# alexncoleman/WeaklySupervisedDL

Hardware: AMD Instinct MI355X
Metric: SegmentationModel train img/s at B=16 256x256 (higher is better)
Workload: dtype f32

## Files before the change

### weaklysuperviseddl_amd/csrc/conv_igemm.hip

```cpp
#include "common.h"

#include <type_traits>
#include <algorithm>
#include <cstdint>
#include <mutex>

typedef float f32x16 __attribute__((ext_vector_type(16)));

namespace {

constexpr int kThreads = 256;

struct ConvSrc {
    const float* x;
    const float* wt;
    const float* x_amax;
    int KH, KW, bh, ch, K, Cin;
    long long x_bs;
    unsigned x_bytes;
};

struct ConvP {
    const float* x;
    const float* wt;
// ... 2182 lines not shown
            }
        }
        __syncthreads();
    }
    float* slab = p.slab + (long long)blockIdx.x * 64 * 147;
#pragma unroll
    for (int r = 0; r < 16; ++r) {
        const int row = (r & 3) + 8 * (r >> 2) + 4 * lh;
        const int n = nt0 * 32 + l31;
        if (n < 147) {
            slab[(long long)row * 147 + n] = acc0[r];
            slab[(long long)(32 + row) * 147 + n] = acc1[r];
        }
        if (third && 128 + l31 < 147) slab[(long long)(wid * 32 + row) * 147 + 128 + l31] = acc2[r];
    }
}

static bool stem_wgrad_eligible(int B, int Cin, int H, int W, int Cout, int kh, int kw, int stride, int pad, int dil) {
    return Cin == 3 && Cout == 64 && kh == 7 && kw == 7 && stride == 2 && pad == 3 && dil == 1 && H >= 7 && W >= 7;
}
static int stem_wgrad_grid(int B, int OH, int OW) {
    const long long tiles = (long long)B * wsdl::cdiv(OH, kSwTH) * wsdl::cdiv(OW, kStemTW);
    return (int)std::min<long long>(tiles, kSwMaxGrid);
}

static size_t wgrad_dys_bytes(int Cout, int Cin, int N, int P) {
    if (!wgrad_chunk32(Cout, Cin, N)) return 0;
    const size_t n = (size_t)wsdl::cdiv(P, 32) * Cout * w2row_bytes(g_conv_arith);
    return n < (1ull << 31) ? n : 0;
}

static int wgrad_bands(int Cout, int Cin, int OW, int W, int kw, int stride, int pad, int dil, Band* bands) {
    int BM, BN;
    bool fast;
    wgrad_tile(Cout, Cin, &BM, &BN, &fast);
    bands[0] = Band{0, OW};
    if (!fast || stride != 1) return 1;
    if (wgrad_chunk32(Cout, Cin, kw * kw * Cin)) return 1;
    return column_bands(OW, W, 1, dil, -pad, 1, kw, bands);
}

size_t wsdl_conv2d_wgrad_presplit_bytes(int B, int Cin, int H, int W, int Cout, int kh, int kw, int stride, int pad, int dil) {
    int OH, OW;
    if (check_geom(B, Cin, H, W, Cout, kh, kw, stride, pad, dil, &OH, &OW)) return 0;
    if (g_conv_arith != 1 && g_conv_arith != 2) return 0;
    if (wgrad_role_swap(Cin, Cout, kh, kw, stride, pad)) return 0;
    const int N = kh * kw * Cin, P = B * OH * OW;
    const size_t bytes = wgrad_dys_bytes(Cout, Cin, N, P);
    if (!bytes || P % 32 != 0) return 0;
    const long long xb = (long long)B * Cin * H * W * 4, dyb = (long long)B * Cout * OH * OW * 4;
    if (xb >= (1ll << 31) || dyb >= (1ll << 31)) return 0;
    bool taps_aligned = true;
    for (int kx = 0; kx < kw; ++kx) taps_aligned = taps_aligned && (((kx * dil - pad) & 3) == 0);
    const bool direct = g_wgrad_direct && taps_aligned && stride == 1 && OW % 32 == 0 && W % 4 == 0 && (H * W) % 4 == 0;
    const bool dyraw = direct && g_wgrad_dyraw && (N / 128 <= 10 || g_wgrad_dyraw == 2) && (OH * OW) % 4 == 0;
    return dyraw ? 0 : bytes;
}

size_t wsdl_conv2d_wgrad_workspace(int B, int Cin, int H, int W, int Cout, int kh, int kw, int stride,
                                   int pad, int dil) {
    int OH, OW;
    if (check_geom(B, Cin, H, W, Cout, kh, kw, stride, pad, dil, &OH, &OW)) return 0;
    if (wgrad_role_swap(Cin, Cout, kh, kw, stride, pad))
        return wsdl::align_up((size_t)Cout * Cin * sizeof(float), 256) +
               wsdl_conv2d_wgrad_workspace(B, Cout, OH, OW, Cin, 1, 1, 1, 0, 1);
    const int N = kh * kw * Cin;
    Band bands[8];
    const int nb = wgrad_bands(Cout, Cin, OW, W, kw, stride, pad, dil, bands);
    const int n_live = __builtin_popcountll(live_taps(H, W, OH, OW, kh, kw, stride, pad, dil)) * Cin;
    size_t slabs = (size_t)nb * wgrad_splits(Cout, Cin, N, B * OH * OW, n_live, wgrad_tap_balance(H, OH, kh, stride, pad, dil)) *
                   Cout * N * sizeof(float);
    if (stem_wgrad_eligible(B, Cin, H, W, Cout, kh, kw, stride, pad, dil))
        slabs = std::max(slabs, (size_t)stem_wgrad_grid(B, OH, OW) * Cout * N * sizeof(float));
    return wsdl::align_up(slabs, 256) + wsdl::align_up(wgrad_dys_bytes(Cout, Cin, N, B * OH * OW), 256) +
           (g_wgrad_chan_scale ? wsdl::align_up((size_t)(Cin + Cout) * sizeof(float), 256) : 0);
}

struct WgradExtra {
    const float* x_chan;
    const float* dy_chan;
    const void* dy_presplit;
};
static int wgrad_impl(const float* x, const float* dy, float* dw, int B, int Cin, int H, int W,
                      int Cout, int kh, int kw, int stride, int pad, int dil, int accumulate,
                      long long x_bs, long long dy_bs, const float* x_amax, const float* dy_amax, void* ws,
                      size_t ws_bytes, wsdl_stream_t stream, WgradExtra ex = WgradExtra{}) {
    WSDL_REQUIRE(x && dy && dw && ws, "conv2d_wgrad: null pointer");
    int OH, OW;
    if (int rc = check_geom(B, Cin, H, W, Cout, kh, kw, stride, pad, dil, &OH, &OW)) return rc;
    if (wgrad_role_swap(Cin, Cout, kh, kw, stride, pad)) {
        const size_t t_bytes = wsdl::align_up((size_t)Cout * Cin * sizeof(float), 256);
        WSDL_REQUIRE(ws_bytes > t_bytes, "conv2d_wgrad: workspace too small");
        float* dwt = static_cast<float*>(ws);
        if (int rc = wgrad_impl(dy, x, dwt, B, Cout, OH, OW, Cin, 1, 1, 1, 0, 1, 0,
                                dy_bs ? dy_bs : (long long)Cout * OH * OW, x_bs ? x_bs : (long long)Cin * H * W,
                                dy_amax, x_amax, static_cast<char*>(ws) + t_bytes, ws_bytes - t_bytes, stream,
                                WgradExtra{ex.dy_chan, ex.x_chan, nullptr}))
            return rc;
        WSDL_TRACE("role-swapped (dW^T) + transpose");
        hipLaunchKernelGGL(transpose_add_kernel, dim3(wsdl::cdiv(Cout, 32), wsdl::cdiv(Cin, 32)), dim3(32, 8), 0,
                           wsdl::as_stream(stream), dwt, dw, Cout, Cin, accumulate);
        WSDL_LAUNCH_CHECK();
        return WSDL_OK;
    }
    WgradP p{};
    p.x = x; p.dy = dy; p.slab = static_cast<float*>(ws);
    p.B = B; p.Cin = Cin; p.H = H; p.W = W; p.Cout = Cout; p.OH = OH; p.OW = OW; p.KH = kh; p.KW = kw;
// ... 37 lines not shown
        return wgrad_reduce_one(rd, s);
    }
    const unsigned long long live_all = live_taps(H, W, OH, OW, kh, kw, stride, pad, dil);
    const int S = wgrad_splits(Cout, Cin, p.N, p.P, __builtin_popcountll(live_all) * Cin, wgrad_tap_balance(H, OH, kh, stride, pad, dil));
    Band bands[8];
    const int nb = wgrad_bands(Cout, Cin, OW, W, kw, stride, pad, dil, bands);
    if (nb == 1) bands[0] = Band{0, OW};
    const int S_total = nb * S;
    p.ow0 = 0; p.own = OW; p.slab0 = 0; p.nb = 1; p.splits = S;
    const size_t need = (size_t)S_total * Cout * p.N * sizeof(float);
    if (ws_bytes < need) {
        wsdl::set_error("conv2d_wgrad: workspace %zu < %zu bytes", ws_bytes, need);
        return WSDL_EWORKSPACE;
    }
    const int chunks = wsdl::cdiv(p.P, 32);
    p.chunks_per_split = wsdl::cdiv(chunks, S);
    hipStream_t s = wsdl::as_stream(stream);
    const long long xb = ((long long)(B - 1) * p.x_bs + (long long)Cin * H * W) * 4;
    const long long dyb = ((long long)(B - 1) * p.dy_bs + (long long)Cout * OH * OW) * 4;
    int tBM, tBN;
    bool fast;
    wgrad_tile(Cout, Cin, &tBM, &tBN, &fast);
    if (fast && (xb >= (1ll << 31) || dyb >= (1ll << 31))) {
        const long long img = std::max((long long)Cin * H * W, (long long)Cout * OH * OW) * 4;
        const long long bs = std::max(p.x_bs, p.dy_bs) * 4;
        WSDL_REQUIRE(B > 1 && img < (1ll << 31), "conv2d_wgrad: a single image of 2 GiB or more is not supported");
        long long per = ((1ll << 31) - 4 - img) / bs + 1;
        if (per < 1) per = 1;
        for (int b0 = 0; b0 < B; b0 += (int)per) {
            const int nb_img = (int)std::min<long long>(per, B - b0);
            if (int rc = wgrad_impl(x + (long long)b0 * p.x_bs, dy + (long long)b0 * p.dy_bs, dw, nb_img, Cin, H, W,
                                    Cout, kh, kw, stride, pad, dil, (accumulate || b0 > 0) ? 1 : 0, p.x_bs, p.dy_bs,
                                    x_amax, dy_amax, ws, ws_bytes, stream, WgradExtra{ex.x_chan, ex.dy_chan, nullptr}))
                return rc;
        }
        return WSDL_OK;
    }
    unsigned long long live_mask = ~0ull;
    {
        const double flops = 2.0 * p.P * (double)Cout * p.N;
        double executed = flops;
        const size_t dys_bytes = fast ? wgrad_dys_bytes(Cout, Cin, p.N, p.P) : 0;
        const size_t dys_off = wsdl::align_up(need, 256);
        const bool chunk32 = dys_bytes && ws_bytes >= dys_off + dys_bytes;
        if (wsdl::prof_enabled() && fast) {
            executed = 0.0;
            for (int i = 0; i < nb; ++i)
                executed += flops * ((double)bands[i].own / OW) *
                            wgrad_executed_fraction(B * OH * bands[i].own, OH, bands[i].ow0, bands[i].own, H, W, kh, kw,
                                                    stride, pad, dil, chunk32 ? 32 : 16);
        }
        bool taps_aligned = true;
        for (int kx = 0; kx < kw; ++kx) taps_aligned = taps_aligned && (((kx * dil - pad) & 3) == 0);
        const bool direct = chunk32 && g_conv_arith && g_wgrad_direct && taps_aligned &&
                            stride == 1 && OW % 32 == 0 && W % 4 == 0 && (H * W) % 4 == 0 && p.x_bs % 4 == 0 &&
                            reinterpret_cast<uintptr_t>(x) % 16 == 0;
        wsdl::ProfScope prof(direct ? WSDL_PROF_WGRAD_SPLIT16D
                                    : chunk32 ? WSDL_PROF_WGRAD_SPLIT32
                                     : fast ? WSDL_PROF_WGRAD_FAST_128x128
                                            : (Cout <= 64 ? WSDL_PROF_WGRAD_64x128 : WSDL_PROF_WGRAD_128x128),
                             s, flops, executed,
                             4.0 * ((double)B * Cin * H * W + (double)p.P * Cout + (double)S_total * Cout * p.N));
        constexpr size_t lds64 = 2 * (64 + 128) * 33 * sizeof(float), lds128 = 2 * (128 + 128) * 33 * sizeof(float);
        static std::once_flag once;
        static hipError_t attr_rc = hipSuccess;
        std::call_once(once, [] {
            attr_rc = hipFuncSetAttribute(reinterpret_cast<const void*>(&conv_wgrad_kernel<64, 128, 1>),
                                          hipFuncAttributeMaxDynamicSharedMemorySize, (int)lds64);
            if (attr_rc == hipSuccess)
                attr_rc = hipFuncSetAttribute(reinterpret_cast<const void*>(&conv_wgrad_kernel<128, 128, 2>),
                                              hipFuncAttributeMaxDynamicSharedMemorySize, (int)lds128);
        });
        WSDL_HIP_CHECK(attr_rc);
        if (fast) {
            p.x_bytes = (unsigned)xb;
            p.dy_bytes = (unsigned)dyb;
            if (chunk32) {
                live_mask = live_all;
                unsigned char* dys = static_cast<unsigned char*>(ws) + dys_off;
                const long long total = 2ll * wsdl::cdiv(p.P, 32) * Cout;
                dim3 grid(p.N / 128, Cout / 128, S);
                p.xcd_order = ((long long)grid.x * grid.y * grid.z) % 8 == 0 ? g_wgrad_xcd : 0;
                const dim3 sgrid((int)std::min<long long>((total + 255) / 256, 16384));
                const size_t cm_off = wsdl::align_up(dys_off + dys_bytes, 256);
                const bool cm_fits = ws_bytes >= cm_off + (size_t)(Cin + Cout) * sizeof(float);
                p.xa_stride = 0;
                int dy_stride = 0;
                if (g_conv_arith) {
                    float* cm = reinterpret_cast<float*>(static_cast<unsigned char*>(ws) + cm_off);
                    if (ex.x_chan) {
                        p.x_amax = x_amax = ex.x_chan;
                        p.xa_stride = 1;
                    } else if (g_wgrad_chan_scale && cm_fits) {
                        WSDL_HIP_CHECK(hipMemsetAsync(cm, 0, (size_t)Cin * sizeof(float), s));
                        hipLaunchKernelGGL(channel_amax_kernel, dim3(Cin, std::min(B, std::max(1, 1024 / Cin))), dim3(256), 0, s, x, B, Cin,
                                           H * W, p.x_bs, cm);
                        WSDL_LAUNCH_CHECK();
                        p.x_amax = x_amax = cm;
                        p.xa_stride = 1;
                    }
                    if (ex.dy_chan) {
                        dy_amax = ex.dy_chan;
                        dy_stride = 1;
                    } else if (g_wgrad_chan_scale && cm_fits) {
                        WSDL_HIP_CHECK(hipMemsetAsync(cm + Cin, 0, (size_t)Cout * sizeof(float), s));
                        hipLaunchKernelGGL(channel_amax_kernel, dim3(Cout, std::min(B, std::max(1, 1024 / Cout))), dim3(256), 0, s, dy, B,
                                           Cout, OH * OW, p.dy_bs, cm + Cin);
                        WSDL_LAUNCH_CHECK();
                        dy_amax = cm + Cin;
                        dy_stride = 1;
                    }
                }
                p.da_stride = dy_stride;
                const bool cs = p.xa_stride || dy_stride;
                const bool presplit = ex.dy_presplit && ex.dy_chan && g_conv_arith;
                if (presplit) dys = static_cast<unsigned char*>(const_cast<void*>(ex.dy_presplit));
                if (g_conv_arith) {
                    WSDL_REQUIRE(x_amax && dy_amax, "conv2d_wgrad: the fp16x2 split kernel needs x_amax and dy_amax");
                    WSDL_TRACE("wgrad_split16%s S=%d xcd=%d cs=%d grid=%ux%ux%u", direct ? "d" : "", S, p.xcd_order, (int)cs, grid.x, grid.y, grid.z);
                    if (direct) {
                        const bool dyraw = !presplit && taps_aligned && g_wgrad_dyraw && (p.N / 128 <= 10 || g_wgrad_dyraw == 2) &&
                                           (OH * OW) % 4 == 0 && p.dy_bs % 4 == 0 &&
                                           reinterpret_cast<uintptr_t>(dy) % 16 == 0 && p.dy_bytes != 0;
                        WSDL_TRACE(dyraw ? "dyraw" : presplit ? "dY pre-split by its producer" : "dy_split16");
                        if (!dyraw && !presplit) {
                            hipLaunchKernelGGL(dy_split16_kernel, sgrid, dim3(256), 0, s, dy, dys, B, Cout, OH * OW, p.dy_bs, p.P, dy_amax,
                                               dy_stride);
                            WSDL_LAUNCH_CHECK();
                        }
                        if (dyraw && cs)
                            hipLaunchKernelGGL((conv_wgrad_split16d_kernel<0, true, true>), grid, dim3(kThreads), 0, s, p, dys,
                                               (unsigned)dys_bytes, dy_amax);
                        else if (dyraw)
                            hipLaunchKernelGGL((conv_wgrad_split16d_kernel<0, true>), grid, dim3(kThreads), 0, s, p, dys,
                                               (unsigned)dys_bytes, dy_amax);
                        else if (cs)
                            hipLaunchKernelGGL((conv_wgrad_split16d_kernel<0, false, true>), grid, dim3(kThreads), 0, s, p, dys,
                                               (unsigned)dys_bytes, dy_amax);
                        else
                            hipLaunchKernelGGL(conv_wgrad_split16d_kernel<0>, grid, dim3(kThreads), 0, s, p, dys,
                                               (unsigned)dys_bytes, dy_amax);
                    } else {
                        WSDL_TRACE(presplit ? "dY pre-split by its producer" : "dy_split16");
                        if (!presplit) {
                            hipLaunchKernelGGL(dy_split16_kernel, sgrid, dim3(256), 0, s, dy, dys, B, Cout, OH * OW, p.dy_bs, p.P, dy_amax,
                                               dy_stride);
                            WSDL_LAUNCH_CHECK();
                        }
                        if (cs)
                            hipLaunchKernelGGL((conv_wgrad_split16_kernel<128, 128, true>), grid, dim3(kThreads), 0, s, p, dys,
                                               (unsigned)dys_bytes, dy_amax);
                        else
                            hipLaunchKernelGGL((conv_wgrad_split16_kernel<128, 128>), grid, dim3(kThreads), 0, s, p, dys,
                                               (unsigned)dys_bytes, dy_amax);
                    }
                } else {
                    WSDL_TRACE("wgrad_split32 bf16x3 S=%d xcd=%d grid=%ux%ux%u", S, p.xcd_order, grid.x, grid.y, grid.z);
                    hipLaunchKernelGGL(dy_split_kernel<0>, sgrid, dim3(256), 0, s, dy, dys, B, Cout, OH * OW, p.dy_bs, p.P,
                                       static_cast<const float*>(nullptr));
                    WSDL_LAUNCH_CHECK();
                    hipLaunchKernelGGL((conv_wgrad_split32_kernel<128, 128, 0>), grid, dim3(kThreads), 0, s, p, dys,
                                       (unsigned)dys_bytes, static_cast<const float*>(nullptr));
                }
            } else {
                WgradP q = p;
                q.nb = nb;
                q.splits = S;
                for (int i = 0; i < nb && nb > 1; ++i) {
                    q.b_ow0[i] = bands[i].ow0;
                    q.b_own[i] = bands[i].own;
                    q.b_cps[i] = wsdl::cdiv(wsdl::cdiv((long long)B * OH * bands[i].own, 32), S);
                }
                int rc;
                WSDL_TRACE("wgrad_fp32_fast<%d,%d> S=%d nb=%d", tBM, tBN, S, nb);
                if (tBM == 128 && tBN == 128) rc = launch_wgrad_fast<128, 128, 2>(q, s, S_total);
                else if (tBM == 128) rc = launch_wgrad_fast<128, 64, 2>(q, s, S_total);
                else if (tBN == 128) rc = launch_wgrad_fast<64, 128, 1>(q, s, S_total);
                else rc = launch_wgrad_fast<64, 64, 2>(q, s, S_total);
                if (rc) return rc;
            }
        } else if (Cout <= 64) {
            WSDL_TRACE("wgrad_fp32_generic<64,128> S=%d", S);
            dim3 grid(wsdl::cdiv(p.N, 128), wsdl::cdiv(Cout, 64), S);
            hipLaunchKernelGGL((conv_wgrad_kernel<64, 128, 1>), grid, dim3(kThreads), lds64, s, p);
        } else {
            WSDL_TRACE("wgrad_fp32_generic<128,128> S=%d", S);
            dim3 grid(wsdl::cdiv(p.N, 128), wsdl::cdiv(Cout, 128), S);
            hipLaunchKernelGGL((conv_wgrad_kernel<128, 128, 2>), grid, dim3(kThreads), lds128, s, p);
        }
    }
    WSDL_LAUNCH_CHECK();
    WgradReduce rd{};
    rd.slab = p.slab; rd.dw = dw; rd.S = S_total; rd.Cout = Cout; rd.Cin = Cin; rd.T = kh * kw; rd.accumulate = accumulate;
    rd.live = live_mask;
    const long long total = (long long)Cout * p.N;
    const int T = kh * kw;
    if (T >= 2 && T <= 16 && Cout <= 65535) {
        rd.kind = WGRAD_REDUCE_TILED;
        rd.grid_x = wsdl::cdiv(Cin, 32);
        rd.nblocks = rd.grid_x * Cout;
    } else if (T == 1 && total % 4 == 0 && (reinterpret_cast<uintptr_t>(dw) & 15) == 0) {
        rd.kind = WGRAD_REDUCE_VEC4;
        rd.nblocks = (int)std::min<long long>((total / 4 + 255) / 256, 8192);
    } else if (S_total >= 64 && total < 64 * 512) {
        rd.kind = WGRAD_REDUCE_MANY16;
        rd.nblocks = (int)((total + 15) / 16);
    } else if (S_total >= 16 && total <= (1ll << 24)) {
// ... 62 lines not shown
```

### weaklysuperviseddl_amd/csrc/conv_split.h

```cpp
#pragma once

typedef __bf16 bf16x8 __attribute__((ext_vector_type(8)));
typedef __bf16 bf16x2 __attribute__((ext_vector_type(2)));
typedef _Float16 half8 __attribute__((ext_vector_type(8)));
typedef float f32x4 __attribute__((ext_vector_type(4)));

__device__ __forceinline__ void split3(float x0, float x1, unsigned& h, unsigned& m, unsigned& l) {
    f32x2 v = {x0, x1};
    h = __builtin_bit_cast(unsigned, __builtin_convertvector(v, bf16x2));
    f32x2 r = {x0 - __builtin_bit_cast(float, h << 16), x1 - __builtin_bit_cast(float, h & 0xffff0000u)};
    m = __builtin_bit_cast(unsigned, __builtin_convertvector(r, bf16x2));
    f32x2 s = {r[0] - __builtin_bit_cast(float, m << 16), r[1] - __builtin_bit_cast(float, m & 0xffff0000u)};
    l = __builtin_bit_cast(unsigned, __builtin_convertvector(s, bf16x2));
}

__device__ __forceinline__ void split2hs(float x0, float x1, unsigned& h, unsigned& l) {
    f32x2 v = {x0, x1};
    const half2v hv = __builtin_convertvector(v, half2v);
    h = __builtin_bit_cast(unsigned, hv);
    f32x2 r = {(x0 - (float)hv[0]) * 2048.f, (x1 - (float)hv[1]) * 2048.f};
    l = __builtin_bit_cast(unsigned, __builtin_convertvector(r, half2v));
}

template <int AR> struct SplitArith;
template <> struct SplitArith<0> {
    static constexpr int NP = 3;
    using frag = bf16x8;
    static __device__ __forceinline__ f32x16 mma(frag a, frag b, f32x16 c) {
        return __builtin_amdgcn_mfma_f32_32x32x16_bf16(a, b, c, 0, 0, 0);
    }
};
template <> struct SplitArith<1> {
    static constexpr int NP = 2;
    using frag = half8;
    static __device__ __forceinline__ f32x16 mma(frag a, frag b, f32x16 c) {
        return __builtin_amdgcn_mfma_f32_32x32x16_f16(a, b, c, 0, 0, 0);
    }
};
template <> struct SplitArith<2> : SplitArith<1> {};
template <int AR, typename F>
__device__ __forceinline__ f32x16 split_products(const F (&a)[SplitArith<AR>::NP], const F (&b)[SplitArith<AR>::NP], f32x16 c) {
    using A = SplitArith<AR>;
    if constexpr (AR == 0) {
        c = A::mma(a[2], b[0], c);
        c = A::mma(a[0], b[2], c);
        c = A::mma(a[1], b[1], c);
        c = A::mma(a[1], b[0], c);
        c = A::mma(a[0], b[1], c);
        c = A::mma(a[0], b[0], c);
    } else {
        c = A::mma(a[1], b[0], c);
        c = A::mma(a[0], b[1], c);
        c = A::mma(a[0], b[0], c);
    }
    return c;
}

constexpr int split_k16_bytes(int AR) { return AR ? 64 : 96; }
__host__ __device__ constexpr long long split_layout_bytes(int AR, long long k_total, long long rows) {
    return (k_total / 16) * rows * split_k16_bytes(AR) + 16;
}

template <int BM, int BN, int WM, int BK, int NT, int AR, bool MF, bool MS, bool IL>
__device__ __forceinline__ void conv_igemm_split_body(const ConvP& p, const int bx_in, const int by_in, const int bz,
                                                      const int grid_x, const int grid_y) {
    static_assert(!MF || (AR >= 1 && BK == 32), "16x16x32 form: fp16x2, K chunk 32");
    using Ar = SplitArith<AR>;
    using frag = typename Ar::frag;
    constexpr int NP = Ar::NP;
    constexpr int K16B = split_k16_bytes(AR);
    constexpr int WN = (NT / 64) / WM;
    constexpr int MI = BM / WM / 32, NI = BN / WN / 32;
    static_assert(MI >= 1 && NI >= 1 && MI * 32 * WM == BM && NI * 32 * WN == BN, "bad tile");
// ... 838 lines not shown

constexpr int kW16Row = 128;

__global__ void dy_split16_kernel(const float* __restrict__ dy, unsigned char* __restrict__ out, int B, int Cout,
                                  int OHOW, long long dy_bs, int P, const float* __restrict__ amax, int amax_stride) {
    const int groups = 2 * ((P + 31) / 32);
    const long long total = (long long)groups * Cout;
    for (long long idx = blockIdx.x * (long long)blockDim.x + threadIdx.x; idx < total;
         idx += (long long)gridDim.x * blockDim.x) {
        const int g = (int)(idx % groups), c = (int)(idx / groups);
        int ex;
        const float sc = pow2_scale(amax[c * amax_stride], ex);
        float v[16];
        const int p0 = g * 16;
        if (p0 >= P) {
#pragma unroll
            for (int e = 0; e < 16; ++e) v[e] = 0.f;
        } else if (OHOW % 16 == 0) {
            const int b = p0 / OHOW, r = p0 - b * OHOW;
            const float4* src = reinterpret_cast<const float4*>(dy + (long long)b * dy_bs + (long long)c * OHOW + r);
#pragma unroll
            for (int e = 0; e < 4; ++e) {
                const float4 q = src[e];
                v[4 * e] = q.x; v[4 * e + 1] = q.y; v[4 * e + 2] = q.z; v[4 * e + 3] = q.w;
            }
        } else {
#pragma unroll
            for (int e = 0; e < 16; ++e) {
                const int pix = p0 + e;
                float t = 0.f;
                if (pix < P) {
                    const int b = pix / OHOW, r = pix - b * OHOW;
                    t = dy[(long long)b * dy_bs + (long long)c * OHOW + r];
                }
                v[e] = t;
            }
        }
        unsigned pc[2][8];
#pragma unroll
        for (int e = 0; e < 8; ++e) split2h(v[2 * e] * sc, v[2 * e + 1] * sc, pc[0][e], pc[1][e]);
        unsigned char* row = out + ((long long)(g >> 1) * Cout + c) * kW16Row;
        const int sw = (c >> 1) & 7;
#pragma unroll
        for (int c2 = 0; c2 < 2; ++c2)
#pragma unroll
            for (int h = 0; h < 2; ++h) {
                const int u = 4 * c2 + 2 * (g & 1) + h;
                *reinterpret_cast<u32x4*>(row + ((u ^ sw) << 4)) =
                    u32x4{pc[c2][4 * h], pc[c2][4 * h + 1], pc[c2][4 * h + 2], pc[c2][4 * h + 3]};
            }
    }
}

template <int BM, int BN, bool CS = false>
__global__ __launch_bounds__(kThreads, 2) void conv_wgrad_split16_kernel(WgradP p, const unsigned char* __restrict__ dys,
                                                                        unsigned dys_bytes, const float* __restrict__ dy_amax) {
    static_assert(BM == 128 && BN == 128, "tile");
    constexpr int BK = 32, ROW = kW16Row;
    constexpr int WN = 2;
    constexpr int TMI = BM / 32, TNI = BN / 32;
    constexpr int A_U = BM * ROW / 16 / kThreads;
    constexpr int B_PER = BN / 8;
    constexpr unsigned kOOB = 0x80000000u;

    __shared__ __attribute__((aligned(16))) unsigned char As[BM * ROW];
    __shared__ __attribute__((aligned(16))) unsigned char Bs[BN * ROW];

    const int tid = threadIdx.x;
    const int lane = tid & 63, wid = tid >> 6;
    const int wm = wid / WN, wn = wid % WN;
    int bx = blockIdx.x, by = blockIdx.y, bz = blockIdx.z;
    if (p.xcd_order) {
        const int gx = gridDim.x, gy = gridDim.y;
        const int L = (bz * gy + by) * gx + bx, eighth = (gx * gy * (int)gridDim.z) >> 3;
        const int Lp = (L & 7) * eighth + (L >> 3);
        bz = Lp / (gx * gy);
        const int r = Lp - bz * (gx * gy);
        by = r / gx;
        bx = r - by * gx;
    }
    const int n0 = bx * BN, m0 = by * BM;
    const int zsplit = bz, w_cps = p.chunks_per_split;
    const int W_P = p.P;
    const int OHOW = p.OH * p.OW, HW = p.H * p.W;
    const int px = tid & 31, hw = tid >> 5;

    const __amdgpu_buffer_rsrc_t rdy =
        __builtin_amdgcn_make_buffer_rsrc(const_cast<unsigned char*>(dys), 0, (int)dys_bytes, 0x00020000);
    const __amdgpu_buffer_rsrc_t rx =
        __builtin_amdgcn_make_buffer_rsrc(const_cast<float*>(p.x), 0, (int)p.x_bytes, 0x00020000);
    int ex = 0, ed = 0;
    float xs = 1.f;
    if constexpr (!CS) {
        xs = pow2_scale(*p.x_amax, ex);
        (void)pow2_scale(*dy_amax, ed);
    }
    const float out_scale = pow2(-(ex + ed));

    const int tap0 = n0 / p.Cin, ci0 = n0 - tap0 * p.Cin;
    const int t_dh = (tap0 / p.KW) * p.dil - p.pad, t_dw = (tap0 % p.KW) * p.dil - p.pad;
    const unsigned b_row = (unsigned)((ci0 + 2 * hw) * HW);
    __shared__ float xst[CS ? BN : 1];
    __shared__ int edy_s[CS ? BM : 1];
    if constexpr (CS) {
        if (tid < BN) {
            int e_;
            xst[tid] = pow2_scale(p.x_amax[(ci0 + tid) * p.xa_stride], e_);
            (void)pow2_scale(dy_amax[(m0 + tid) * p.da_stride], e_);
            edy_s[tid] = e_;
        }
        __syncthreads();
    }
    const float* xsr = xst + 2 * hw + (px & 1);

    unsigned voff_a[A_U];
#pragma unroll
    for (int e = 0; e < A_U; ++e) voff_a[e] = (unsigned)(m0 * ROW + (tid + e * kThreads) * 16);

    f32x4 acc[TMI][TNI];
#pragma unroll
    for (int i = 0; i < TMI; ++i)
#pragma unroll
        for (int j = 0; j < TNI; ++j) acc[i][j] = f32x4{0.f, 0.f, 0.f, 0.f};

    u32x4 ra[2][A_U];
    unsigned rb[2][B_PER];
    const int chunk_begin = zsplit * w_cps;
    const int total_chunks = (W_P + BK - 1) / BK;
    const int chunk_end = min(chunk_begin + w_cps, total_chunks);

    const bool row_chunks = (p.OW % BK) == 0;
    unsigned nvb = kOOB;
    auto decode = [&](int c) {
        nvb = kOOB;
        if (row_chunks) {
            const int first = c * BK;
            const int grow = first / p.OW, ow = first - grow * p.OW + px;
            const int pb = grow / p.OH, oh = grow - pb * p.OH;
            const int ih = oh * p.stride + t_dh, iw = ow * p.stride + t_dw;
            if (ih >= 0 && ih < p.H && iw >= 0 && iw < p.W)
                nvb = ((unsigned)((long long)pb * p.x_bs) + (unsigned)(ih * p.W) + (unsigned)iw + b_row) * 4u;
            return;
        }
        const int pix = c * BK + px;
        if (pix < W_P) {
            const int pb = pix / OHOW, rr = pix - pb * OHOW;
            const int oh = rr / p.OW, ow = rr - oh * p.OW;
            const int ih = oh * p.stride + t_dh, iw = ow * p.stride + t_dw;
            if (ih >= 0 && ih < p.H && iw >= 0 && iw < p.W)
                nvb = ((unsigned)((long long)pb * p.x_bs) + (unsigned)(ih * p.W + iw) + b_row) * 4u;
        }
    };
    auto next_valid = [&](int c) {
        for (; c < chunk_end; ++c) {
            decode(c);
            if (__any(nvb != kOOB)) break;
        }
        return c;
    };
    auto load_tiles = [&](auto slot_c, int c) {
        constexpr int S = decltype(slot_c)::value;
        const unsigned soff_a = (unsigned)c * (unsigned)(p.Cout * ROW);
#pragma unroll
        for (int e = 0; e < A_U; ++e) ra[S][e] = __builtin_amdgcn_raw_buffer_load_b128(rdy, voff_a[e], soff_a, 0);
#pragma unroll
        for (int e = 0; e < B_PER; ++e)
            rb[S][e] = __builtin_amdgcn_raw_buffer_load_b32(rx, nvb, (unsigned)(((e & 1) + 16 * (e >> 1)) * HW) * 4u, 0);
    };
    const bool even = (px & 1) == 0;
    const int pair = px >> 1;
    const unsigned st_row = (unsigned)((2 * hw + (even ? 0 : 1)) * ROW + (pair & 3) * 4);
    const unsigned st_u0 = (unsigned)((((pair >> 2)) ^ (hw & 7)) << 4), st_u1 = (unsigned)(((4 + (pair >> 2)) ^ (hw & 7)) << 4);
    auto store_tiles = [&](auto slot_c) {
        constexpr int S = decltype(slot_c)::value;
#pragma unroll
        for (int e = 0; e < A_U; ++e) *reinterpret_cast<u32x4*>(As + (tid + e * kThreads) * 16) = ra[S][e];
#pragma unroll
        for (int i = 0; i < B_PER / 2; ++i) {
            const unsigned give = even ? rb[S][2 * i + 1] : rb[S][2 * i];
            const unsigned recv = (unsigned)__builtin_amdgcn_mov_dpp((int)give, 0xB1, 0xF, 0xF, true);
            const unsigned x0 = even ? rb[S][2 * i] : recv;
            const unsigned x1 = even ? recv : rb[S][2 * i + 1];
            unsigned ph, pl;
            const float xsc = CS ? xsr[CS ? 16 * i : 0] : xs;
            split2h(__builtin_bit_cast(float, x0) * xsc, __builtin_bit_cast(float, x1) * xsc, ph, pl);
            unsigned char* d = Bs + st_row + i * 16 * ROW;
            *reinterpret_cast<unsigned*>(d + st_u0) = ph;
            *reinterpret_cast<unsigned*>(d + st_u1) = pl;
        }
    };

    const int l15 = lane & 15, lg = lane >> 4;
    const unsigned fr0 = (unsigned)(l15 * ROW + ((lg ^ (l15 >> 1)) << 4)), fr1 = (unsigned)(l15 * ROW + (((4 + lg) ^ (l15 >> 1)) << 4));
    const unsigned char* Ab = As + wm * (BM / 2) * ROW;
    const unsigned char* Bb = Bs + wn * (BN / 2) * ROW;
    if (t_dh >= p.H || (p.OH - 1) * p.stride + t_dh < 0 || t_dw >= p.W || (p.OW - 1) * p.stride + t_dw < 0) return;
    using S0 = std::integral_constant<int, 0>;
    using S1 = std::integral_constant<int, 1>;
    int c0 = next_valid(chunk_begin), c1 = chunk_end;
    if (c0 < chunk_end) {
        load_tiles(S0{}, c0);
        c1 = next_valid(c0 + 1);
        if (c1 < chunk_end) load_tiles(S1{}, c1);
    }
    auto step = [&](auto slot_c) {
        int c2 = chunk_end;
        store_tiles(slot_c);
        if (c1 < chunk_end) c2 = next_valid(c1 + 1);
        if (c2 < chunk_end) load_tiles(slot_c, c2);
        lds_barrier();
        half8 a[TMI][2], b[TNI][2];
#pragma unroll
        for (int i = 0; i < TMI; ++i) {
            a[i][0] = *reinterpret_cast<const half8*>(Ab + i * 16 * ROW + fr0);
            a[i][1] = *reinterpret_cast<const half8*>(Ab + i * 16 * ROW + fr1);
        }
#pragma unroll
        for (int j = 0; j < TNI; ++j) {
            b[j][0] = *reinterpret_cast<const half8*>(Bb + j * 16 * ROW + fr0);
            b[j][1] = *reinterpret_cast<const half8*>(Bb + j * 16 * ROW + fr1);
        }
#pragma unroll
        for (int i = 0; i < TMI; ++i)
#pragma unroll
            for (int j = 0; j < TNI; ++j) {
                f32x4 c = acc[i][j];
                c = __builtin_amdgcn_mfma_f32_16x16x32_f16(a[i][1], b[j][0], c, 0, 0, 0);
                c = __builtin_amdgcn_mfma_f32_16x16x32_f16(a[i][0], b[j][1], c, 0, 0, 0);
                c = __builtin_amdgcn_mfma_f32_16x16x32_f16(a[i][0], b[j][0], c, 0, 0, 0);
                acc[i][j] = c;
            }
        lds_barrier();
        c0 = c1;
        c1 = c2;
    };
    while (c0 < chunk_end) {
        step(S0{});
        if (c0 >= chunk_end) break;
        step(S1{});
    }

    float* slab = p.slab + (long long)(p.slab0 + bz) * p.Cout * p.N;
    if constexpr (CS) {
        int en[TNI];
#pragma unroll
        for (int j = 0; j < TNI; ++j) (void)pow2_scale(p.x_amax[(ci0 + wn * (BN / 2) + j * 16 + l15) * p.xa_stride], en[j]);
#pragma unroll
        for (int i = 0; i < TMI; ++i)
#pragma unroll
            for (int r = 0; r < 4; ++r) {
                const int row = wm * (BM / 2) + i * 16 + lg * 4 + r, co = m0 + row;
                const int edr = edy_s[row];
#pragma unroll
                for (int j = 0; j < TNI; ++j)
                    slab[(long long)co * p.N + n0 + wn * (BN / 2) + j * 16 + l15] = ldexpf(acc[i][j][r], -(en[j] + edr));
            }
        return;
    }
#pragma unroll
    for (int i = 0; i < TMI; ++i)
#pragma unroll
        for (int j = 0; j < TNI; ++j) {
            const int n = n0 + wn * (BN / 2) + j * 16 + l15;
#pragma unroll
            for (int r = 0; r < 4; ++r) {
                const int co = m0 + wm * (BM / 2) + i * 16 + lg * 4 + r;
                slab[(long long)co * p.N + n] = acc[i][j][r] * out_scale;
            }
        }
}

template <int MODE, bool DYRAW = false, bool CS = false>
__global__ __launch_bounds__(kThreads, 2) void conv_wgrad_split16d_kernel(WgradP p, const unsigned char* __restrict__ dys,
                                                                         unsigned dys_bytes, const float* __restrict__ dy_amax) {
    constexpr int BM = 128, BN = 128, BK = 32, ROW = kW16Row;
    constexpr int TMI = BM / 16, TNI = 2;
    constexpr int A_U = BM * ROW / 16 / kThreads;
    __shared__ __attribute__((aligned(16))) unsigned char As[2][BM * ROW];

    const int tid = threadIdx.x;
    const int lane = tid & 63, wid = tid >> 6;
    int bx = blockIdx.x, by = blockIdx.y, bz = blockIdx.z;
    if (p.xcd_order) {
        const int gx = gridDim.x, gy = gridDim.y;
        const int L = (bz * gy + by) * gx + bx, eighth = (gx * gy * (int)gridDim.z) >> 3;
        const int Lp = (L & 7) * eighth + (L >> 3);
        bz = Lp / (gx * gy);
        const int r = Lp - bz * (gx * gy);
        by = r / gx;
        bx = r - by * gx;
    }
    const int n0 = bx * BN, m0 = by * BM;
    const int HW = p.H * p.W;
    const __amdgpu_buffer_rsrc_t rdy =
        __builtin_amdgcn_make_buffer_rsrc(const_cast<unsigned char*>(dys), 0, (int)dys_bytes, 0x00020000);
    const __amdgpu_buffer_rsrc_t rx =
        __builtin_amdgcn_make_buffer_rsrc(const_cast<float*>(p.x), 0, (int)p.x_bytes, 0x00020000);
    int ex = 0, ed = 0;
    float xs = 1.f, ds = 1.f;
    if constexpr (!CS) {
        xs = pow2_scale(*p.x_amax, ex);
        ds = pow2_scale(*dy_amax, ed);
    }
    const float out_scale = pow2(-(ex + ed));
    const __amdgpu_buffer_rsrc_t rdr =
        __builtin_amdgcn_make_buffer_rsrc(const_cast<float*>(p.dy), 0, (int)p.dy_bytes, 0x00020000);
    const int OHOW_ = p.OH * p.OW;
    const int dr_row = tid >> 3, dr_q = tid & 7;

    const int tap0 = n0 / p.Cin, ci0 = n0 - tap0 * p.Cin;
    const int t_dh = (tap0 / p.KW) * p.dil - p.pad, t_dw = (tap0 % p.KW) * p.dil - p.pad;
    if (t_dh >= p.H || (p.OH - 1) + t_dh < 0 || t_dw >= p.W || (p.OW - 1) + t_dw < 0) return;
    const int l15 = lane & 15, lg = lane >> 4;
    unsigned vrow[TNI];
#pragma unroll
    for (int j = 0; j < TNI; ++j) vrow[j] = (unsigned)((ci0 + wid * 32 + j * 16 + l15) * HW + lg * 8);
    float xsr[CS ? TNI : 1], dsr[CS && DYRAW ? A_U : 1];
    int exr[CS ? TNI : 1];
    __shared__ int edy_s[CS ? BM : 1];
    if constexpr (CS) {
        if (tid < BM) {
            int e_;
            (void)pow2_scale(dy_amax[(m0 + tid) * p.da_stride], e_);
            edy_s[tid] = e_;
        }
        __syncthreads();
#pragma unroll
        for (int j = 0; j < TNI; ++j) xsr[j] = pow2_scale(p.x_amax[(ci0 + wid * 32 + j * 16 + l15) * p.xa_stride], exr[j]);
        if constexpr (DYRAW) {
#pragma unroll
            for (int e = 0; e < A_U; ++e) {
                int e_;
                dsr[e] = pow2_scale(dy_amax[(m0 + dr_row + 32 * e) * p.da_stride], e_);
            }
        }
    }

    unsigned voff_a[A_U];
#pragma unroll
    for (int e = 0; e < A_U; ++e) voff_a[e] = (unsigned)(m0 * ROW + (tid + e * kThreads) * 16);

    f32x4 acc[TMI][TNI];
#pragma unroll
    for (int i = 0; i < TMI; ++i)
#pragma unroll
        for (int j = 0; j < TNI; ++j) acc[i][j] = f32x4{0.f, 0.f, 0.f, 0.f};

    const int chunk_begin = bz * p.chunks_per_split;
    const int total_chunks = (p.P + BK - 1) / BK;
    const int chunk_end = min(chunk_begin + p.chunks_per_split, total_chunks);
    const int cpr = p.OW / BK;

    int c_iw0 = 0;
    long long c_base = 0, c_dy = 0;
    auto decode = [&](int c) {
        const int grow = c / cpr, ow0 = (c - grow * cpr) * BK;
        const int pb = grow / p.OH, oh = grow - pb * p.OH;
        const int ih = oh + t_dh;
        c_iw0 = ow0 + t_dw;
        c_base = (long long)pb * p.x_bs + (long long)ih * p.W + c_iw0;
        c_dy = (long long)pb * p.dy_bs + (long long)oh * p.OW + ow0;
        return ih >= 0 && ih < p.H && c_iw0 + BK > 0 && c_iw0 < p.W;
    };
    auto next_valid = [&](int c) {
        for (; c < chunk_end; ++c)
            if (decode(c)) break;
        return c;
    };
    auto run = [&](auto sh_c) {
        constexpr int SH = decltype(sh_c)::value;
        u32x4 ra[2][A_U];
        u32x4 rbx[2][TNI][3];
        int ld_iw0[2] = {0, 0};
        auto load_tiles = [&](auto slot_c, int c) {
            constexpr int S = decltype(slot_c)::value;
            if constexpr (DYRAW) {
                const unsigned db = (unsigned)((c_dy + (long long)(m0 + dr_row) * OHOW_ + dr_q * 4) * 4ll);
#pragma unroll
                for (int e = 0; e < A_U; ++e)
                    ra[S][e] = __builtin_amdgcn_raw_buffer_load_b128(rdr, db + (unsigned)(e * 32 * OHOW_) * 4u, 0, 0);
            } else {
                const unsigned soff_a = (unsigned)c * (unsigned)(p.Cout * ROW);
#pragma unroll
                for (int e = 0; e < A_U; ++e) ra[S][e] = __builtin_amdgcn_raw_buffer_load_b128(rdy, voff_a[e], soff_a, 0);
            }
            const unsigned cb = (unsigned)(c_base * 4ll);
#pragma unroll
            for (int j = 0; j < TNI; ++j) {
                const unsigned vo = vrow[j] * 4u + cb - (unsigned)(SH * 4);
                rbx[S][j][0] = __builtin_amdgcn_raw_buffer_load_b128(rx, vo, 0, 0);
                rbx[S][j][1] = __builtin_amdgcn_raw_buffer_load_b128(rx, vo + 16u, 0, 0);
                if constexpr (SH != 0) rbx[S][j][2] = __builtin_amdgcn_raw_buffer_load_b128(rx, vo + 32u, 0, 0);
            }
            ld_iw0[S] = c_iw0;
        };
        auto store_a = [&](auto slot_c, int buf) {
            constexpr int S = decltype(slot_c)::value;
            if constexpr (DYRAW) {
#pragma unroll
                for (int e = 0; e < A_U; ++e) {
                    const int r = dr_row + 32 * e;
                    const unsigned u0 = ra[S][e][0], u1 = ra[S][e][1], u2 = ra[S][e][2], u3 = ra[S][e][3];
                    unsigned h0, l0, h1, l1;
                    const float dsc = CS ? dsr[CS ? e : 0] : ds;
                    split2h(__builtin_bit_cast(float, u0) * dsc, __builtin_bit_cast(float, u1) * dsc, h0, l0);
                    split2h(__builtin_bit_cast(float, u2) * dsc, __builtin_bit_cast(float, u3) * dsc, h1, l1);
                    const unsigned sw = (unsigned)((r >> 1) & 7);
                    unsigned char* row = As[buf] + r * ROW + (dr_q & 1) * 8;
                    *reinterpret_cast<u32x2*>(row + ((((unsigned)(dr_q >> 1)) ^ sw) << 4)) = u32x2{h0, h1};
                    *reinterpret_cast<u32x2*>(row + (((4u + (unsigned)(dr_q >> 1)) ^ sw) << 4)) = u32x2{l0, l1};
                }
            } else {
#pragma unroll
                for (int e = 0; e < A_U; ++e) *reinterpret_cast<u32x4*>(As[buf] + (tid + e * kThreads) * 16) = ra[S][e];
            }
        };
        const unsigned fr0 = (unsigned)(l15 * ROW + ((lg ^ (l15 >> 1)) << 4)), fr1 = (unsigned)(l15 * ROW + (((4 + lg) ^ (l15 >> 1)) << 4));
        using S0 = std::integral_constant<int, 0>;
        using S1 = std::integral_constant<int, 1>;

        int c0 = next_valid(chunk_begin), c1 = chunk_end;
        int buf = 0;
        if (c0 < chunk_end) {
            load_tiles(S0{}, c0);
            c1 = next_valid(c0 + 1);
            if (c1 < chunk_end) load_tiles(S1{}, c1);
            store_a(S0{}, 0);
        }
        auto step = [&](auto slot_c) {
            constexpr int S = decltype(slot_c)::value;
            half8 b[TNI][2];
            {
                const int first = ld_iw0[S] + lg * 8;
                const int lo = -first, hi = p.W - first;
#pragma unroll
                for (int j = 0; j < TNI; ++j) {
                    unsigned d[12];
#pragma unroll
                    for (int e = 0; e < 4; ++e) {
                        d[e] = rbx[S][j][0][e];
                        d[4 + e] = rbx[S][j][1][e];
                        d[8 + e] = SH != 0 ? rbx[S][j][2][e] : 0u;
                    }
                    float v[8];
#pragma unroll
                    for (int e = 0; e < 8; ++e) {
                        const unsigned u = d[e + SH];
                        v[e] = __builtin_bit_cast(float, u);
                    }
                    u32x4 ph, pl;
                    const float xsc = CS ? xsr[CS ? j : 0] : xs;
#pragma unroll
                    for (int e = 0; e < 4; ++e) {
                        const float x0 = (2 * e >= lo && 2 * e < hi) ? v[2 * e] * xsc : 0.f;
                        const float x1 = (2 * e + 1 >= lo && 2 * e + 1 < hi) ? v[2 * e + 1] * xsc : 0.f;
                        unsigned h, l;
                        split2h(x0, x1, h, l);
                        ph[e] = h;
                        pl[e] = l;
                    }
                    b[j][0] = __builtin_bit_cast(half8, ph);
                    b[j][1] = __builtin_bit_cast(half8, pl);
                }
            }
            int c2 = chunk_end;
            if (c1 < chunk_end) c2 = next_valid(c1 + 1);
            if (c2 < chunk_end) load_tiles(slot_c, c2);
            lds_barrier();
            const unsigned char* Ab = As[buf];
#pragma unroll
            for (int i = 0; i < TMI; ++i) {
                const half8 a0 = *reinterpret_cast<const half8*>(Ab + i * 16 * ROW + fr0);
                const half8 a1 = *reinterpret_cast<const half8*>(Ab + i * 16 * ROW + fr1);
#pragma unroll
                for (int j = 0; j < TNI; ++j) {
                    f32x4 c = acc[i][j];
                    c = __builtin_amdgcn_mfma_f32_16x16x32_f16(a1, b[j][0], c, 0, 0, 0);
                    c = __builtin_amdgcn_mfma_f32_16x16x32_f16(a0, b[j][1], c, 0, 0, 0);
                    c = __builtin_amdgcn_mfma_f32_16x16x32_f16(a0, b[j][0], c, 0, 0, 0);
                    acc[i][j] = c;
                }
            }
            if (c1 < chunk_end) store_a(std::integral_constant<int, 1 - S>{}, buf ^ 1);
            buf ^= 1;
            c0 = c1;
            c1 = c2;
        };
        while (c0 < chunk_end) {
            step(S0{});
            if (c0 >= chunk_end) break;
            step(S1{});
        }
    };
    static_assert(MODE == 0, "only the aligned loop is instantiated (the misaligned-tap loops were removed in round 4)");
    run(std::integral_constant<int, 0>{});

    float* slab = p.slab + (long long)(p.slab0 + bz) * p.Cout * p.N;
    if constexpr (CS) {
#pragma unroll
        for (int i = 0; i < TMI; ++i)
#pragma unroll
            for (int r = 0; r < 4; ++r) {
                const int row = i * 16 + lg * 4 + r, co = m0 + row;
                const int edr = edy_s[row];
#pragma unroll
                for (int j = 0; j < TNI; ++j)
                    slab[(long long)co * p.N + n0 + wid * 32 + j * 16 + l15] = ldexpf(acc[i][j][r], -(exr[j] + edr));
            }
        return;
    }
#pragma unroll
    for (int i = 0; i < TMI; ++i)
#pragma unroll
        for (int j = 0; j < TNI; ++j) {
            const int n = n0 + wid * 32 + j * 16 + l15;
#pragma unroll
            for (int r = 0; r < 4; ++r) {
                const int co = m0 + i * 16 + lg * 4 + r;
                slab[(long long)co * p.N + n] = acc[i][j][r] * out_scale;
            }
// ... 3 lines not shown
```

Measured before the change: 897.7.

## Add lean wgrad split16 kernel variants with incremental chunk walking

Adds a LEAN template variant to the weight-gradient split16 kernels. It replaces per-chunk division-based decode with an incrementally stepped row/image walker, and drops the per-element column bounds tests when the taps are unshifted or OW==32. The fp16 hi/lo split moves to a packed f32x2 multiply-subtract form. The lean path is chosen at launch from the geometry and can be turned off with a bit in g_wgrad_direct. The goal is to cut scalar address arithmetic and VALU work in the inner loops, at the cost of more kernel instantiations and subtle boundary-correctness risk.

```diff
diff --git a/weaklysuperviseddl_amd/csrc/conv_igemm.hip b/weaklysuperviseddl_amd/csrc/conv_igemm.hip
--- a/weaklysuperviseddl_amd/csrc/conv_igemm.hip
+++ b/weaklysuperviseddl_amd/csrc/conv_igemm.hip
@@ -2258,7 +2258,7 @@
     if (xb >= (1ll << 31) || dyb >= (1ll << 31)) return 0;
     bool taps_aligned = true;
     for (int kx = 0; kx < kw; ++kx) taps_aligned = taps_aligned && (((kx * dil - pad) & 3) == 0);
-    const bool direct = g_wgrad_direct && taps_aligned && stride == 1 && OW % 32 == 0 && W % 4 == 0 && (H * W) % 4 == 0;
+    const bool direct = (g_wgrad_direct & 1) && taps_aligned && stride == 1 && OW % 32 == 0 && W % 4 == 0 && (H * W) % 4 == 0;
     const bool dyraw = direct && g_wgrad_dyraw && (N / 128 <= 10 || g_wgrad_dyraw == 2) && (OH * OW) % 4 == 0;
     return dyraw ? 0 : bytes;
 }
@@ -2402,7 +2402,9 @@
         }
         bool taps_aligned = true;
         for (int kx = 0; kx < kw; ++kx) taps_aligned = taps_aligned && (((kx * dil - pad) & 3) == 0);
-        const bool direct = chunk32 && g_conv_arith && g_wgrad_direct && taps_aligned &&
+        bool taps_unshifted = true;
+        for (int kx = 0; kx < kw; ++kx) taps_unshifted = taps_unshifted && kx * dil - pad == 0;
+        const bool direct = chunk32 && g_conv_arith && (g_wgrad_direct & 1) && taps_aligned &&
                             stride == 1 && OW % 32 == 0 && W % 4 == 0 && (H * W) % 4 == 0 && p.x_bs % 4 == 0 &&
                             reinterpret_cast<uintptr_t>(x) % 16 == 0;
         wsdl::ProfScope prof(direct ? WSDL_PROF_WGRAD_SPLIT16D
@@ -2467,7 +2469,14 @@
                 if (presplit) dys = static_cast<unsigned char*>(const_cast<void*>(ex.dy_presplit));
                 if (g_conv_arith) {
                     WSDL_REQUIRE(x_amax && dy_amax, "conv2d_wgrad: the fp16x2 split kernel needs x_amax and dy_amax");
-                    WSDL_TRACE("wgrad_split16%s S=%d xcd=%d cs=%d grid=%ux%ux%u", direct ? "d" : "", S, p.xcd_order, (int)cs, grid.x, grid.y, grid.z);
+                    using L0 = std::integral_constant<int, 0>;
+                    using L1 = std::integral_constant<int, 1>;
+                    using L2 = std::integral_constant<int, 2>;
+                    const int lean = (g_wgrad_direct & 2) ? 0
+                                     : direct ? (taps_unshifted && OW == W ? 1 : OW == 32 ? 2 : 0)
+                                              : (OW == 32 ? 1 : 0);
+                    WSDL_TRACE("wgrad_split16%s S=%d xcd=%d cs=%d grid=%ux%ux%u lean=%d", direct ? "d" : "", S, p.xcd_order, (int)cs, grid.x, grid.y,
+                               grid.z, lean);
                     if (direct) {
                         const bool dyraw = !presplit && taps_aligned && g_wgrad_dyraw && (p.N / 128 <= 10 || g_wgrad_dyraw == 2) &&
                                            (OH * OW) % 4 == 0 && p.dy_bs % 4 == 0 &&
@@ -2478,18 +2487,24 @@
                                                dy_stride);
                             WSDL_LAUNCH_CHECK();
                         }
-                        if (dyraw && cs)
-                            hipLaunchKernelGGL((conv_wgrad_split16d_kernel<0, true, true>), grid, dim3(kThreads), 0, s, p, dys,
-                                               (unsigned)dys_bytes, dy_amax);
-                        else if (dyraw)
-                            hipLaunchKernelGGL((conv_wgrad_split16d_kernel<0, true>), grid, dim3(kThreads), 0, s, p, dys,
-                                               (unsigned)dys_bytes, dy_amax);
-                        else if (cs)
-                            hipLaunchKernelGGL((conv_wgrad_split16d_kernel<0, false, true>), grid, dim3(kThreads), 0, s, p, dys,
-                                               (unsigned)dys_bytes, dy_amax);
-                        else
-                            hipLaunchKernelGGL(conv_wgrad_split16d_kernel<0>, grid, dim3(kThreads), 0, s, p, dys,
-                                               (unsigned)dys_bytes, dy_amax);
+                        auto launch = [&](auto lean_c) {
+                            constexpr int L = decltype(lean_c)::value;
+                            if (dyraw && cs)
+                                hipLaunchKernelGGL((conv_wgrad_split16d_kernel<0, true, true, L>), grid, dim3(kThreads), 0, s, p, dys,
+                                                   (unsigned)dys_bytes, dy_amax);
+                            else if (dyraw)
+                                hipLaunchKernelGGL((conv_wgrad_split16d_kernel<0, true, false, L>), grid, dim3(kThreads), 0, s, p, dys,
+                                                   (unsigned)dys_bytes, dy_amax);
+                            else if (cs)
+                                hipLaunchKernelGGL((conv_wgrad_split16d_kernel<0, false, true, L>), grid, dim3(kThreads), 0, s, p, dys,
+                                                   (unsigned)dys_bytes, dy_amax);
+                            else
+                                hipLaunchKernelGGL((conv_wgrad_split16d_kernel<0, false, false, L>), grid, dim3(kThreads), 0, s, p, dys,
+                                                   (unsigned)dys_bytes, dy_amax);
+                        };
+                        if (lean == 1) launch(L1{});
+                        else if (lean == 2) launch(L2{});
+                        else launch(L0{});
                     } else {
                         WSDL_TRACE(presplit ? "dY pre-split by its producer" : "dy_split16");
                         if (!presplit) {
@@ -2497,12 +2512,17 @@
                                                dy_stride);
                             WSDL_LAUNCH_CHECK();
                         }
-                        if (cs)
-                            hipLaunchKernelGGL((conv_wgrad_split16_kernel<128, 128, true>), grid, dim3(kThreads), 0, s, p, dys,
-                                               (unsigned)dys_bytes, dy_amax);
-                        else
-                            hipLaunchKernelGGL((conv_wgrad_split16_kernel<128, 128>), grid, dim3(kThreads), 0, s, p, dys,
-                                               (unsigned)dys_bytes, dy_amax);
+                        auto launch = [&](auto lean_c) {
+                            constexpr bool L = decltype(lean_c)::value != 0;
+                            if (cs)
+                                hipLaunchKernelGGL((conv_wgrad_split16_kernel<128, 128, true, L>), grid, dim3(kThreads), 0, s, p, dys,
+                                                   (unsigned)dys_bytes, dy_amax);
+                            else
+                                hipLaunchKernelGGL((conv_wgrad_split16_kernel<128, 128, false, L>), grid, dim3(kThreads), 0, s, p, dys,
+                                                   (unsigned)dys_bytes, dy_amax);
+                        };
+                        if (lean) launch(L1{});
+                        else launch(L0{});
                     }
                 } else {
                     WSDL_TRACE("wgrad_split32 bf16x3 S=%d xcd=%d grid=%ux%ux%u", S, p.xcd_order, grid.x, grid.y, grid.z);
diff --git a/weaklysuperviseddl_amd/csrc/conv_split.h b/weaklysuperviseddl_amd/csrc/conv_split.h
--- a/weaklysuperviseddl_amd/csrc/conv_split.h
+++ b/weaklysuperviseddl_amd/csrc/conv_split.h
@@ -19,6 +19,14 @@
     const half2v hv = __builtin_convertvector(v, half2v);
     h = __builtin_bit_cast(unsigned, hv);
     f32x2 r = {(x0 - (float)hv[0]) * 2048.f, (x1 - (float)hv[1]) * 2048.f};
+    l = __builtin_bit_cast(unsigned, __builtin_convertvector(r, half2v));
+}
+
+__device__ __forceinline__ void split2h_pk(float x0, float x1, float s, unsigned& h, unsigned& l) {
+    const f32x2 v = f32x2{x0, x1} * f32x2{s, s};
+    const half2v hv = __builtin_convertvector(v, half2v);
+    h = __builtin_bit_cast(unsigned, hv);
+    const f32x2 r = v - __builtin_convertvector(hv, f32x2);
     l = __builtin_bit_cast(unsigned, __builtin_convertvector(r, half2v));
 }
 
@@ -963,7 +971,7 @@
     }
 }
 
-template <int BM, int BN, bool CS = false>
+template <int BM, int BN, bool CS = false, bool LEAN = false>
 __global__ __launch_bounds__(kThreads, 2) void conv_wgrad_split16_kernel(WgradP p, const unsigned char* __restrict__ dys,
                                                                         unsigned dys_bytes, const float* __restrict__ dy_amax) {
     static_assert(BM == 128 && BN == 128, "tile");
@@ -1062,7 +1070,32 @@
                 nvb = ((unsigned)((long long)pb * p.x_bs) + (unsigned)(ih * p.W + iw) + b_row) * 4u;
         }
     };
+    int w_oh = 0;
+    unsigned w_x = 0;
+    const unsigned w_row = (unsigned)(p.stride * p.W) * 4u;
+    const unsigned w_img = (unsigned)((p.x_bs - (long long)p.OH * p.stride * p.W) * 4ll);
+    const int w_iw = px * p.stride + t_dw;
+    const bool w_col = w_iw >= 0 && w_iw < p.W;
+    const bool w_any = __any(w_col);
+    const unsigned w_lane = ((unsigned)w_iw + b_row) * 4u;
     auto next_valid = [&](int c) {
+        if constexpr (LEAN) {
+            if (c == chunk_begin) {
+                const int pb = c / p.OH;
+                w_oh = c - pb * p.OH;
+                w_x = (unsigned)(((long long)pb * p.x_bs + (long long)(w_oh * p.stride + t_dh) * p.W) * 4ll);
+            } else {
+                w_x += w_row;
+                if (++w_oh == p.OH) { w_oh = 0; w_x += w_img; }
+            }
+            for (; c < chunk_end; ++c) {
+                if (w_any && (unsigned)(w_oh * p.stride + t_dh) < (unsigned)p.H) break;
+                w_x += w_row;
+                if (++w_oh == p.OH) { w_oh = 0; w_x += w_img; }
+            }
+            nvb = w_col ? w_lane + w_x : kOOB;
+            return c;
+        }
         for (; c < chunk_end; ++c) {
             decode(c);
             if (__any(nvb != kOOB)) break;
@@ -1094,7 +1127,10 @@
             const unsigned x1 = even ? recv : rb[S][2 * i + 1];
             unsigned ph, pl;
             const float xsc = CS ? xsr[CS ? 16 * i : 0] : xs;
-            split2h(__builtin_bit_cast(float, x0) * xsc, __builtin_bit_cast(float, x1) * xsc, ph, pl);
+            if constexpr (LEAN)
+                split2h_pk(__builtin_bit_cast(float, x0), __builtin_bit_cast(float, x1), xsc, ph, pl);
+            else
+                split2h(__builtin_bit_cast(float, x0) * xsc, __builtin_bit_cast(float, x1) * xsc, ph, pl);
             unsigned char* d = Bs + st_row + i * 16 * ROW;
             *reinterpret_cast<unsigned*>(d + st_u0) = ph;
             *reinterpret_cast<unsigned*>(d + st_u1) = pl;
@@ -1181,12 +1217,13 @@
         }
 }
 
-template <int MODE, bool DYRAW = false, bool CS = false>
+template <int MODE, bool DYRAW = false, bool CS = false, int LEAN = 0>
 __global__ __launch_bounds__(kThreads, 2) void conv_wgrad_split16d_kernel(WgradP p, const unsigned char* __restrict__ dys,
                                                                          unsigned dys_bytes, const float* __restrict__ dy_amax) {
     constexpr int BM = 128, BN = 128, BK = 32, ROW = kW16Row;
     constexpr int TMI = BM / 16, TNI = 2;
     constexpr int A_U = BM * ROW / 16 / kThreads;
+    constexpr unsigned kOOB = 0x80000000u;
     __shared__ __attribute__((aligned(16))) unsigned char As[2][BM * ROW];
 
     const int tid = threadIdx.x;
@@ -1273,20 +1310,68 @@
         c_dy = (long long)pb * p.dy_bs + (long long)oh * p.OW + ow0;
         return ih >= 0 && ih < p.H && c_iw0 + BK > 0 && c_iw0 < p.W;
     };
+    int w_oh = 0, w_cb = 0;
+    unsigned w_x = 0, w_dy = 0;
+    const unsigned w_row = (unsigned)(p.W - p.OW) * 4u;
+    const unsigned w_img_x = (unsigned)((p.x_bs - (long long)p.OH * p.W) * 4ll);
+    const unsigned w_img_dy = (unsigned)((p.dy_bs - (long long)p.OH * p.OW) * 4ll);
+    auto w_seek = [&](int c) {
+        const int grow = c / cpr, pb = grow / p.OH;
+        w_cb = c - grow * cpr;
+        w_oh = grow - pb * p.OH;
+        w_x = (unsigned)(((long long)pb * p.x_bs + (long long)(w_oh + t_dh) * p.W + w_cb * BK + t_dw) * 4ll);
+        w_dy = (unsigned)(((long long)pb * p.dy_bs + (long long)w_oh * p.OW + w_cb * BK) * 4ll);
+    };
+    auto w_step = [&]() {
+        w_x += BK * 4u;
+        w_dy += BK * 4u;
+        if (LEAN == 2 || ++w_cb == cpr) {
+            w_cb = 0;
+            w_x += w_row;
+            if (++w_oh == p.OH) {
+                w_oh = 0;
+                w_x += w_img_x;
+                w_dy += w_img_dy;
+            }
+        }
+    };
     auto next_valid = [&](int c) {
+        if constexpr (LEAN != 0) {
+            if (c == chunk_begin) w_seek(c); else w_step();
+            for (; c < chunk_end && (unsigned)(w_oh + t_dh) >= (unsigned)p.H; ++c) w_step();
+            return c;
+        }
         for (; c < chunk_end; ++c)
             if (decode(c)) break;
         return c;
     };
+    bool w_in[2] = {true, true};
+    if constexpr (LEAN == 2) {
+#pragma unroll
+        for (int q = 0; q < 2; ++q) w_in[q] = (unsigned)(t_dw + lg * 8 + q * 4) < (unsigned)p.W;
+    }
+    unsigned dyrow4 = 0;
+    if constexpr (DYRAW) dyrow4 = (unsigned)(((long long)(m0 + dr_row) * OHOW_ + dr_q * 4) * 4ll);
     auto run = [&](auto sh_c) {
         constexpr int SH = decltype(sh_c)::value;
         u32x4 ra[2][A_U];
         u32x4 rbx[2][TNI][3];
         int ld_iw0[2] = {0, 0};
-        auto load_tiles = [&](auto slot_c, int c) {
+        auto load_tiles = [&](auto slot_c, int c, bool live = true) {
             constexpr int S = decltype(slot_c)::value;
+            if constexpr (LEAN != 0) {
+                const unsigned cb = w_x;
+#pragma unroll
+                for (int j = 0; j < TNI; ++j) {
+                    static_assert(SH == 0, "a load is one 4-column group");
+                    const unsigned vo = vrow[j] * 4u + cb;
+                    rbx[S][j][0] = __builtin_amdgcn_raw_buffer_load_b128(rx, live && w_in[0] ? vo : kOOB, 0, 0);
+                    rbx[S][j][1] = __builtin_amdgcn_raw_buffer_load_b128(rx, live && w_in[1] ? vo + 16u : kOOB, 0, 0);
+                }
+                if (!live) return;
+            }
             if constexpr (DYRAW) {
-                const unsigned db = (unsigned)((c_dy + (long long)(m0 + dr_row) * OHOW_ + dr_q * 4) * 4ll);
+                const unsigned db = LEAN != 0 ? dyrow4 + w_dy : (unsigned)((c_dy + (long long)(m0 + dr_row) * OHOW_ + dr_q * 4) * 4ll);
 #pragma unroll
                 for (int e = 0; e < A_U; ++e)
                     ra[S][e] = __builtin_amdgcn_raw_buffer_load_b128(rdr, db + (unsigned)(e * 32 * OHOW_) * 4u, 0, 0);
@@ -1295,6 +1380,7 @@
 #pragma unroll
                 for (int e = 0; e < A_U; ++e) ra[S][e] = __builtin_amdgcn_raw_buffer_load_b128(rdy, voff_a[e], soff_a, 0);
             }
+            if constexpr (LEAN != 0) return;
             const unsigned cb = (unsigned)(c_base * 4ll);
 #pragma unroll
             for (int j = 0; j < TNI; ++j) {
@@ -1314,8 +1400,13 @@
                     const unsigned u0 = ra[S][e][0], u1 = ra[S][e][1], u2 = ra[S][e][2], u3 = ra[S][e][3];
                     unsigned h0, l0, h1, l1;
                     const float dsc = CS ? dsr[CS ? e : 0] : ds;
-                    split2h(__builtin_bit_cast(float, u0) * dsc, __builtin_bit_cast(float, u1) * dsc, h0, l0);
-                    split2h(__builtin_bit_cast(float, u2) * dsc, __builtin_bit_cast(float, u3) * dsc, h1, l1);
+                    if constexpr (LEAN != 0) {
+                        split2h_pk(__builtin_bit_cast(float, u0), __builtin_bit_cast(float, u1), dsc, h0, l0);
+                        split2h_pk(__builtin_bit_cast(float, u2), __builtin_bit_cast(float, u3), dsc, h1, l1);
+                    } else {
+                        split2h(__builtin_bit_cast(float, u0) * dsc, __builtin_bit_cast(float, u1) * dsc, h0, l0);
+                        split2h(__builtin_bit_cast(float, u2) * dsc, __builtin_bit_cast(float, u3) * dsc, h1, l1);
+                    }
                     const unsigned sw = (unsigned)((r >> 1) & 7);
                     unsigned char* row = As[buf] + r * ROW + (dr_q & 1) * 8;
                     *reinterpret_cast<u32x2*>(row + ((((unsigned)(dr_q >> 1)) ^ sw) << 4)) = u32x2{h0, h1};
@@ -1335,7 +1426,7 @@
         if (c0 < chunk_end) {
             load_tiles(S0{}, c0);
             c1 = next_valid(c0 + 1);
-            if (c1 < chunk_end) load_tiles(S1{}, c1);
+            if (LEAN != 0 || c1 < chunk_end) load_tiles(S1{}, c1, c1 < chunk_end);
             store_a(S0{}, 0);
         }
         auto step = [&](auto slot_c) {
@@ -1363,10 +1454,14 @@
                     const float xsc = CS ? xsr[CS ? j : 0] : xs;
 #pragma unroll
                     for (int e = 0; e < 4; ++e) {
-                        const float x0 = (2 * e >= lo && 2 * e < hi) ? v[2 * e] * xsc : 0.f;
-                        const float x1 = (2 * e + 1 >= lo && 2 * e + 1 < hi) ? v[2 * e + 1] * xsc : 0.f;
                         unsigned h, l;
-                        split2h(x0, x1, h, l);
+                        if constexpr (LEAN != 0) {
+                            split2h_pk(v[2 * e], v[2 * e + 1], xsc, h, l);
+                        } else {
+                            const float x0 = (2 * e >= lo && 2 * e < hi) ? v[2 * e] * xsc : 0.f;
+                            const float x1 = (2 * e + 1 >= lo && 2 * e + 1 < hi) ? v[2 * e + 1] * xsc : 0.f;
+                            split2h(x0, x1, h, l);
+                        }
                         ph[e] = h;
                         pl[e] = l;
                     }
@@ -1376,7 +1471,7 @@
             }
             int c2 = chunk_end;
             if (c1 < chunk_end) c2 = next_valid(c1 + 1);
-            if (c2 < chunk_end) load_tiles(slot_c, c2);
+            if (LEAN != 0 || c2 < chunk_end) load_tiles(slot_c, c2, c2 < chunk_end);
             lds_barrier();
             const unsigned char* Ab = As[buf];
 #pragma unroll
```

After: 906.5, median of 6. No clear change (+1.0%).
